# hiroyasuakada/EgoRear

Measured on AMD Instinct MI355X. Metric: 4-view frames/sec (heatmap+MVFEx+3D lift), higher is better.
Workload: dtype f32 (fp16x2 split, 22-bit operands, fp32 accumulate)

## Files before the change

egorear_amd/csrc/egr_pointwise.hip:

```cpp
#include "egr_common.h"
#include <stdlib.h>

namespace {

__global__ __launch_bounds__(256) void maxpool_kernel(const float* x, float* y, int n, int h, int w, int c4, int ho,
                                                      int wo, int k, int stride, int pad) {
    int64_t idx = (int64_t)blockIdx.x * 256 + threadIdx.x;
    int64_t total = (int64_t)n * ho * wo * c4;
    if (idx >= total) return;
    int cq = (int)(idx % c4);
    int64_t p = idx / c4;
    int ox = (int)(p % wo);
    p /= wo;
    int oy = (int)(p % ho);
    int img = (int)(p / ho);
    f32x4 best = {-INFINITY, -INFINITY, -INFINITY, -INFINITY};
    for (int dy = 0; dy < k; ++dy) {
        int iy = oy * stride - pad + dy;
        if (iy < 0 || iy >= h) continue;
        for (int dx = 0; dx < k; ++dx) {
            int ix = ox * stride - pad + dx;
            if (ix < 0 || ix >= w) continue;
            f32x4 v = *reinterpret_cast<const f32x4*>(x + (((int64_t)img * h + iy) * w + ix) * (c4 * 4) + cq * 4);
            best[0] = fmaxf(best[0], v[0]);
// ... 194 lines not shown
    int64_t r = idx / c;
    int jj = (int)(r % j), bb = (int)(r / j);
    if (bpg > 0) embed += (int64_t)(bb / bpg) * j * c;
    y[idx] = (embed[jj * c + ch] + bfb[(int64_t)bb * c + ch]) + hm_embed[idx];
}

__global__ __launch_bounds__(256) void tokens_to_nhwc_kernel(const float* x, float* y, int b, int j, int hw) {
    int64_t idx = (int64_t)blockIdx.x * 256 + threadIdx.x;
    if (idx >= (int64_t)b * j * hw) return;
    int jj = (int)(idx % j);
    int64_t r = idx / j;
    int p = (int)(r % hw), bb = (int)(r / hw);
    y[idx] = x[((int64_t)bb * j + jj) * hw + p];
}


#ifndef HT_ROWS
#define HT_ROWS 8
#endif
constexpr int HT_H = HT_ROWS, HT_W = 32, HT_SRC_H = HT_ROWS / 2 + 2, HT_SRC_W = 18, HT_MAXCO = 16, HT_MAXCIN = 128;
constexpr int HT_RPW = HT_H / 4, HT_NG = 2 * HT_RPW;
typedef float f32x4_mfma __attribute__((ext_vector_type(4)));

template <int CIN>
__global__ __launch_bounds__(256) void up2_relu_head_kernel(const float* lo, int h, int w, int cin_rt, const float* wgt, const float* bias,
                                                            int cout, float* planes, egr_nmap map, int npg, int64_t gy) {
    extern __shared__ __attribute__((aligned(16))) float s_src[];
    const int cin = CIN > 0 ? CIN : cin_rt;
    const int ld = cin + 4;
    const int ho = 2 * h, wo = 2 * w;
    const int tiles_x = wo / HT_W, tiles_y = ho / HT_H;
    int t = blockIdx.x;
    const int img = t / (tiles_x * tiles_y);
    t -= img * tiles_x * tiles_y;
    const int ty = t / tiles_x, tx = t - ty * tiles_x;
    const int oy0 = ty * HT_H, ox0 = tx * HT_W;
    const int grp = img / npg;
    const float sh = (ho > 1) ? (float)(h - 1) / (float)(ho - 1) : 0.f;
    const float sw = (wo > 1) ? (float)(w - 1) / (float)(wo - 1) : 0.f;
    const int sy0 = (int)(sh * (float)oy0), sx0 = (int)(sw * (float)ox0);
    const int c4n = cin >> 2;
    const float* src = lo + (int64_t)img * h * w * cin;
    constexpr int NLD = (HT_SRC_H * HT_SRC_W * (HT_MAXCIN / 4) + 255) / 256;
    f32x4 stg[NLD];
    const int nsrc = HT_SRC_H * HT_SRC_W * c4n;
#pragma unroll
    for (int u = 0; u < NLD; ++u) {
        const int i = threadIdx.x + 256 * u;
        const int ii = i < nsrc ? i : 0;
// ... 52 lines not shown
        }
    };
    const int kblocks = ksteps >> 2;
    fetch(0, 0);
#pragma unroll
    for (int j = 0; j < HT_MAXCIN / 16; ++j) {
        if (j < kblocks) {
            if (j + 1 < kblocks) fetch(j + 1, (j + 1) & 1);
            __builtin_amdgcn_sched_barrier(0);
            f32x4 u[HT_NG];
#pragma unroll
            for (int mg = 0; mg < HT_NG; ++mg) {
                const f32x4* v = sv[j & 1][mg];
                u[mg] = wy0[mg] * (wx0[mg] * v[0] + wx1[mg] * v[1]) + wy1[mg] * (wx0[mg] * v[2] + wx1[mg] * v[3]);
            }
#pragma unroll
            for (int r = 0; r < 4; ++r)
#pragma unroll
                for (int mg = 0; mg < HT_NG; ++mg)
                    acc[mg] = __builtin_amdgcn_mfma_f32_16x16x4f32(fmaxf(u[mg][r], 0.f), bw[4 * j + r], acc[mg], 0, 0, 0);
            __builtin_amdgcn_sched_barrier(0);
        }
    }
    if (pj < cout) {
#pragma unroll
        for (int mg = 0; mg < HT_NG; ++mg) {
            const int oy = oy0 + HT_RPW * wave + (mg >> 1);
            const int oxg = ox0 + (mg & 1) * 16;
            f32x4 v = {acc[mg][0] + bco, acc[mg][1] + bco, acc[mg][2] + bco, acc[mg][3] + bco};
            *reinterpret_cast<f32x4*>(outg + (int64_t)pj * ho * wo + (int64_t)oy * wo + oxg + 4 * kq) = v;
        }
    }
}

constexpr int PT_H = 8, PT_W = 32, PT_SRC_H = PT_H / 2 + 2, PT_SRC_W = 18, PT_NG = 2;
__global__ __launch_bounds__(512) void up2_relu_head_p_kernel(const float* lo, int h, int w, const float* wgt, const float* bias, int cout,
                                                              float* planes, egr_nmap map, int npg, int64_t gy, int ntiles) {
    constexpr int CIN = 128, LD = CIN + 4, C4N = CIN / 4;
    extern __shared__ __attribute__((aligned(16))) float s_src[];
    const int ho = 2 * h, wo = 2 * w;
    const int tiles_x = wo / PT_W, tiles_y = ho / PT_H;
    const float sh = (ho > 1) ? (float)(h - 1) / (float)(ho - 1) : 0.f;
    const float sw = (wo > 1) ? (float)(w - 1) / (float)(wo - 1) : 0.f;
    constexpr int NSRC = PT_SRC_H * PT_SRC_W * C4N;
    constexpr int NLD = (NSRC + 511) / 512;
    f32x4 stg[NLD];
    const int lane = threadIdx.x & 63, wave = threadIdx.x >> 6;
    const int pj = lane & 15, kq = lane >> 4;
    auto decode = [&](int t, int& img, int& oy0, int& ox0) {
        img = t / (tiles_x * tiles_y);
        t -= img * tiles_x * tiles_y;
        const int ty = t / tiles_x, tx = t - ty * tiles_x;
        oy0 = ty * PT_H;
        ox0 = tx * PT_W;
    };
    auto request = [&](int t) {
        int img, oy0, ox0;
        decode(t, img, oy0, ox0);
        const int sy0 = (int)(sh * (float)oy0), sx0 = (int)(sw * (float)ox0);
        const float* src = lo + (int64_t)img * h * w * CIN;
#pragma unroll
        for (int u = 0; u < NLD; ++u) {
            const int i = threadIdx.x + 512 * u;
            const int ii = i < NSRC ? i : 0;
            const int cq = ii % C4N, p = ii / C4N;
            const int py = p / PT_SRC_W, px = p - py * PT_SRC_W;
            const int iy = min(sy0 + py, h - 1), ix = min(sx0 + px, w - 1);
            stg[u] = *reinterpret_cast<const f32x4*>(src + ((int64_t)iy * w + ix) * CIN + cq * 4);
        }
    };
    float bw[CIN / 4];
    float bco = 0.f;
    int cur_grp = -1;
    int tile = blockIdx.x;
    if (tile < ntiles) request(tile);
    for (; tile < ntiles; tile += gridDim.x) {
#pragma unroll
        for (int u = 0; u < NLD; ++u) {
            const int i = threadIdx.x + 512 * u;
            if (i < NSRC) {
                const int cq = i % C4N, p = i / C4N;
                *reinterpret_cast<f32x4*>(&s_src[p * LD + cq * 4]) = stg[u];
            }
        }
        __syncthreads();
        if (tile + (int)gridDim.x < ntiles) request(tile + gridDim.x);
        int img, oy0, ox0;
        decode(tile, img, oy0, ox0);
        const int grp = img / npg;
        if (grp != cur_grp) {
            cur_grp = grp;
            const float* wg = wgt + (int64_t)grp * cout * CIN;
#pragma unroll
            for (int s_ = 0; s_ < CIN / 4; ++s_) bw[s_] = pj < cout ? wg[pj * CIN + 16 * (s_ >> 2) + 4 * kq + (s_ & 3)] : 0.f;
            bco = (bias && pj < cout) ? bias[grp * cout + pj] : 0.f;
        }
        const int sy0 = (int)(sh * (float)oy0), sx0 = (int)(sw * (float)ox0);
        float* outg = planes + grp * gy + egr_map(map, img - grp * npg);
        const float* q00[PT_NG]; const float* q01[PT_NG]; const float* q10[PT_NG]; const float* q11[PT_NG];
        float wy0[PT_NG], wy1[PT_NG], wx0[PT_NG], wx1[PT_NG];
#pragma unroll
        for (int mg = 0; mg < PT_NG; ++mg) {
            const int oy = oy0 + wave;
            const int ox = ox0 + mg * 16 + pj;
            const float fy = sh * (float)oy, fx = sw * (float)ox;
            const int y0 = (int)fy, x0 = (int)fx;
            const int y1 = min(y0 + 1, h - 1), x1 = min(x0 + 1, w - 1);
            wy1[mg] = fminf(fmaxf(fy - (float)y0, 0.f), 1.f); wx1[mg] = fminf(fmaxf(fx - (float)x0, 0.f), 1.f);
            wy0[mg] = 1.f - wy1[mg]; wx0[mg] = 1.f - wx1[mg];
            q00[mg] = s_src + ((y0 - sy0) * PT_SRC_W + (x0 - sx0)) * LD + 4 * kq;
            q01[mg] = s_src + ((y0 - sy0) * PT_SRC_W + (x1 - sx0)) * LD + 4 * kq;
            q10[mg] = s_src + ((y1 - sy0) * PT_SRC_W + (x0 - sx0)) * LD + 4 * kq;
            q11[mg] = s_src + ((y1 - sy0) * PT_SRC_W + (x1 - sx0)) * LD + 4 * kq;
        }
        f32x4_mfma acc[PT_NG];
#pragma unroll
        for (int mg = 0; mg < PT_NG; ++mg) acc[mg] = f32x4_mfma{0.f, 0.f, 0.f, 0.f};
        f32x4 sv[2][PT_NG][4];
        auto fetch = [&](int j, int par) {
#pragma unroll
            for (int mg = 0; mg < PT_NG; ++mg) {
                sv[par][mg][0] = *reinterpret_cast<const f32x4*>(q00[mg] + 16 * j);
                sv[par][mg][1] = *reinterpret_cast<const f32x4*>(q01[mg] + 16 * j);
                sv[par][mg][2] = *reinterpret_cast<const f32x4*>(q10[mg] + 16 * j);
                sv[par][mg][3] = *reinterpret_cast<const f32x4*>(q11[mg] + 16 * j);
            }
        };
        fetch(0, 0);
#pragma unroll
        for (int j = 0; j < CIN / 16; ++j) {
            if (j + 1 < CIN / 16) fetch(j + 1, (j + 1) & 1);
            __builtin_amdgcn_sched_barrier(0);
            f32x4 u[PT_NG];
#pragma unroll
            for (int mg = 0; mg < PT_NG; ++mg) {
                const f32x4* v = sv[j & 1][mg];
                u[mg] = wy0[mg] * (wx0[mg] * v[0] + wx1[mg] * v[1]) + wy1[mg] * (wx0[mg] * v[2] + wx1[mg] * v[3]);
            }
#pragma unroll
            for (int r = 0; r < 4; ++r)
#pragma unroll
                for (int mg = 0; mg < PT_NG; ++mg)
                    acc[mg] = __builtin_amdgcn_mfma_f32_16x16x4f32(fmaxf(u[mg][r], 0.f), bw[4 * j + r], acc[mg], 0, 0, 0);
            __builtin_amdgcn_sched_barrier(0);
        }
        if (pj < cout) {
#pragma unroll
            for (int mg = 0; mg < PT_NG; ++mg) {
                const int oy = oy0 + wave;
                const int oxg = ox0 + mg * 16;
                f32x4 v = {acc[mg][0] + bco, acc[mg][1] + bco, acc[mg][2] + bco, acc[mg][3] + bco};
                *reinterpret_cast<f32x4*>(outg + (int64_t)pj * ho * wo + (int64_t)oy * wo + oxg + 4 * kq) = v;
            }
        }
        __syncthreads();
    }
}

inline unsigned nblocks(int64_t total) { return (unsigned)((total + 255) / 256); }

}

extern "C" int egr_maxpool_nhwc_f32(const float* x, float* y, int32_t n, int32_t h, int32_t w, int32_t c, int32_t k,
                                    int32_t stride, int32_t pad, void* stream) {
    if (!x || !y) return EGR_ENULL;
    if (n <= 0 || c % 4 != 0 || k <= 0 || stride <= 0 || pad < 0 || 2 * pad > k) return EGR_EINVAL;
    int ho = (h + 2 * pad - k) / stride + 1, wo = (w + 2 * pad - k) / stride + 1;
    int64_t total = (int64_t)n * ho * wo * (c / 4);
    if (total <= 0 || total >= (1LL << 31) * 256) return EGR_EINVAL;
    hipLaunchKernelGGL(maxpool_kernel, dim3(nblocks(total)), dim3(256), 0, (hipStream_t)stream, x, y, n, h, w, c / 4, ho,
                       wo, k, stride, pad);
    return egr_launch_status();
}

extern "C" int egr_upsample2x_nhwc_f32(const float* x, int32_t ldx, float* y, int32_t ldy, int32_t n, int32_t h,
                                       int32_t w, int32_t c, int32_t relu, void* stream) {
    if (!x || !y) return EGR_ENULL;
    if (n <= 0 || h <= 0 || w <= 0 || c % 4 != 0 || ldx % 4 != 0 || ldy % 4 != 0 || ldx < c || ldy < c) return EGR_EINVAL;
    const int c4 = c / 4;
    int c4_shift = 0;
    while ((1 << c4_shift) < c4) ++c4_shift;
    if ((1 << c4_shift) != c4) c4_shift = -1;
    if (2 * h > 65535 || (int64_t)h * w * ldx >= (1LL << 31) || (int64_t)2 * w * c4 >= (1LL << 31)) return EGR_EINVAL;
    static const double nt_mb = getenv("EGR_NT_STORE_MB") ? atof(getenv("EGR_NT_STORE_MB")) : 256.0;
    const int nt = ((double)n * 4 * h * w * c * 4.0 >= nt_mb * 1e6) ? 1 : 0;
    for (int n0 = 0; n0 < n; n0 += 65535) {
        const int nn = n - n0 < 65535 ? n - n0 : 65535;
        hipLaunchKernelGGL(upsample2x_kernel, dim3((unsigned)((2 * w * c4 + 255) / 256), (unsigned)h, (unsigned)nn), dim3(256), 0,
                           (hipStream_t)stream, x + (int64_t)n0 * h * w * ldx, ldx, y + (int64_t)n0 * 4 * h * w * ldy, ldy, nn, h, w, c4, c4_shift, relu, nt);
    }
    return egr_launch_status();
}

static int g_head_persist = getenv("EGR_HEAD_PERSIST") ? atoi(getenv("EGR_HEAD_PERSIST")) != 0 : 1;
extern "C" int egr_head_set_persist(int on) {
    const int old = g_head_persist;
    if (on >= 0) g_head_persist = on != 0;
    return old;
}

extern "C" int egr_up2_relu_head_f32(const float* lo, int32_t n, int32_t h, int32_t w, int32_t cin, const float* wgt, const float* bias,
                                     int32_t cout, float* planes, int32_t n_inner, int64_t stride_inner, int64_t stride_outer,
                                     int32_t groups, int64_t gy, void* stream) {
    if (!lo || !wgt || !planes) return EGR_ENULL;
    if (n <= 0 || groups <= 0 || n % groups != 0 || h <= 0 || w <= 0 || cin <= 0 || cin % 16 != 0 || cin > HT_MAXCIN || cout <= 0 ||
        cout > HT_MAXCO || (2 * h) % HT_H != 0 || (2 * w) % HT_W != 0 || n_inner <= 0 || ((uintptr_t)planes & 15) ||
        ((stride_inner | stride_outer | gy) % 4 != 0))
        return EGR_EINVAL;
    egr_nmap map{n_inner, stride_inner, stride_outer};
    const size_t lds = (size_t)(HT_SRC_H * HT_SRC_W * (cin + 4)) * sizeof(float);
    const int64_t blocks = (int64_t)n * ((2 * h) / HT_H) * ((2 * w) / HT_W);
    if (blocks >= (1LL << 31) || lds > 64 * 1024) return EGR_EINVAL;
    if (g_head_persist && cin == 128 && (2 * h) % PT_H == 0 && (2 * w) % PT_W == 0) {
        const int64_t nt = (int64_t)n * ((2 * h) / PT_H) * ((2 * w) / PT_W);
        int dev = 0, cus = 0;
        if (nt >= 1024 && nt < (1LL << 31) && hipGetDevice(&dev) == hipSuccess && dev >= 0 && dev < 64 &&
            hipDeviceGetAttribute(&cus, hipDeviceAttributeMultiprocessorCount, dev) == hipSuccess && cus > 0) {
            const size_t lds_p = (size_t)(PT_SRC_H * PT_SRC_W * (128 + 4)) * sizeof(float);
            static bool allowed[64] = {};
            if (!allowed[dev]) {
                if (hipFuncSetAttribute(reinterpret_cast<const void*>(up2_relu_head_p_kernel), hipFuncAttributeMaxDynamicSharedMemorySize, (int)lds_p) !=
                    hipSuccess)
                    return EGR_EINVAL;
                allowed[dev] = true;
            }
            const unsigned grid = (unsigned)(nt < cus ? nt : cus);
            hipLaunchKernelGGL(up2_relu_head_p_kernel, dim3(grid), dim3(512), lds_p, (hipStream_t)stream, lo, h, w, wgt, bias, cout, planes, map,
                               n / groups, gy, (int)nt);
            return egr_launch_status();
        }
    }
    if (cin == 128)
        hipLaunchKernelGGL(up2_relu_head_kernel<128>, dim3((unsigned)blocks), dim3(256), lds, (hipStream_t)stream, lo, h, w, cin, wgt, bias, cout,
                           planes, map, n / groups, gy);
    else
        hipLaunchKernelGGL(up2_relu_head_kernel<0>, dim3((unsigned)blocks), dim3(256), lds, (hipStream_t)stream, lo, h, w, cin, wgt, bias, cout,
                           planes, map, n / groups, gy);
    return egr_launch_status();
}

__global__ __launch_bounds__(256) void absmax_kernel(const float* __restrict__ x, int64_t n4, int64_t n, unsigned* __restrict__ rec) {
    float m = 0.f;
    const int64_t stride = (int64_t)gridDim.x * 256;
    int64_t i = (int64_t)blockIdx.x * 256 + threadIdx.x;
    for (; i + 7 * stride < n4; i += 8 * stride) {
        f32x4 v[8];
#pragma unroll
        for (int u = 0; u < 8; ++u) v[u] = *reinterpret_cast<const f32x4*>(x + 4 * (i + u * stride));
#pragma unroll
        for (int u = 0; u < 8; ++u) m = fmaxf(m, fmaxf(fmaxf(fabsf(v[u][0]), fabsf(v[u][1])), fmaxf(fabsf(v[u][2]), fabsf(v[u][3]))));
    }
    for (; i < n4; i += stride) {
        const f32x4 v = *reinterpret_cast<const f32x4*>(x + 4 * i);
        m = fmaxf(fmaxf(m, fmaxf(fabsf(v[0]), fabsf(v[1]))), fmaxf(fabsf(v[2]), fabsf(v[3])));
    }
    if (blockIdx.x == 0 && threadIdx.x < (int)(n - 4 * n4)) m = fmaxf(m, fabsf(x[4 * n4 + threadIdx.x]));
    __shared__ float s_m[4];
    m = wave_max(m);
    if ((threadIdx.x & 63) == 0) s_m[threadIdx.x >> 6] = m;
    __syncthreads();
// ... 98 lines not shown
```

egorear_amd/engine.py:

```python
from __future__ import annotations

import math
import os
import threading
from typing import Dict, Optional, Sequence

import numpy as np
import torch
import torch.nn as nn

from . import hip
from .hip import ACT_GELU, ACT_NONE, ACT_RELU, RES_AFTER_ACT, RES_BEFORE_ACT, RES_NONE, RES_UP2_BEFORE_ACT, Img, NMap

_WORKSPACE_FLOATS = 16 << 20



class PConv:
    __slots__ = ("w", "scale", "shift", "cout", "cin", "kh", "kw", "stride", "pad", "groups")


W6_MAX_ELEMS = 1 << 24


# ... 296 lines not shown
                relu2 = k + 1 < len(m0) and isinstance(m0[k + 1], nn.ReLU)
                end = k + (2 if relu2 else 1)
                fin = end >= len(m0)
                ok = (not up) or relu2
                if up and end + 1 == len(m0) and last_kw and "out_nchw" in last_kw:
                    ok = False
                    ph = st.get(nxt, lambda k=k: pack_convs([g[k] for g in mods]))
                    if relu2 and hip.chain_eligible(x, p.w, ph.w, p.cout, ph.cout, p.groups, p.scale, ph.scale):
                        pre_lo = hip.conv1x1_chain(x, p.w, ph.w, p.cout, ph.cout, shift1=p.shift, shift2=ph.shift, act1=act, act2=ACT_NONE,
                                                   groups=p.groups, amax_out=st.new_amax())
                        i = j
                        continue
                if fin and last_kw:
                    ok = False
                p2 = st.get(nxt, lambda k=k: pack_convs([g[k] for g in mods])) if ok else None
                if ok and hip.chain_eligible(x, p.w, p2.w, p.cout, p2.cout, p.groups, p.scale, p2.scale):
                    y = hip.conv1x1_chain(x, p.w, p2.w, p.cout, p2.cout, shift1=p.shift, shift2=p2.shift, act1=act,
                                          act2=ACT_NONE if up else (ACT_RELU if relu2 else ACT_NONE), groups=p.groups,
                                          out=out if (fin and not up) else None, amax_out=st.new_amax())
                    x = hip.upsample2x(y, out=out if fin else None, relu=True) if up else y
                    i = end
                    continue
            kw = dict(last_kw or {}) if last else {}
            if last and out is not None:
                kw["out"] = out
            x = conv(st, x, p, act, **kw)
            i += 2 if act else 1
        elif isinstance(m, nn.Upsample):
            nxt = m0[i + 1] if i + 1 < len(m0) else None
            if (isinstance(nxt, nn.Conv2d) and nxt.kernel_size == (1, 1) and nxt.stride == (1, 1) and i + 2 < len(m0)
                    and isinstance(m0[i + 2], nn.ReLU)):
                p = st.get(nxt, lambda i=i: pack_convs([g[i + 1] for g in mods]))
                lo, pre_lo = (pre_lo, None) if pre_lo is not None else (conv(st, x, p, ACT_NONE), None)
                fin = m0[i + 3] if i + 4 == len(m0) else None
                if (isinstance(fin, nn.Conv2d) and fin.kernel_size == (1, 1) and fin.stride == (1, 1) and fin.out_channels <= 16
                        and fin.in_channels <= 128 and fin.in_channels % 16 == 0 and last_kw is not None and "out_nchw" in last_kw and (2 * lo.h) % 8 == 0
                        and (2 * lo.w) % 32 == 0):
                    wf = st.get((id(fin), "plain"), lambda i=i: (
                        torch.stack([g[i + 3].weight.detach().float().reshape(fin.out_channels, fin.in_channels) for g in mods]).contiguous(),
                        torch.stack([g[i + 3].bias.detach().float() for g in mods]).contiguous() if fin.bias is not None else None))
                    hip.up2_relu_head(lo, wf[0], wf[1], last_kw["out_nchw"], last_kw["ymap"], last_kw.get("gy", 0), groups=len(mods))
                    return None
                last = (i + 3) >= len(m0)
                x = hip.upsample2x(lo, out=out if last else None, relu=True)
                i += 3
            else:
                x = hip.upsample2x(x)
                i += 1
        elif isinstance(m, nn.MaxPool2d):
            k = m.kernel_size if isinstance(m.kernel_size, int) else m.kernel_size[0]
            s = m.stride if isinstance(m.stride, int) else m.stride[0]
            pd = m.padding if isinstance(m.padding, int) else m.padding[0]
            x = hip.maxpool(x, k, s, pd)
            i += 1
        else:
            raise RuntimeError(f"egorear_amd.run_stack: unexpected module {type(m).__name__}")
    return x



def _pack_stems(trunks) -> tuple:
    wps, scs, shs = [], [], []
    for t in trunks:
        conv1, bn = t.layer_s2[0], t.layer_s2[1]
# ... 269 lines not shown
        P.q = {"w_hp2": pk(stk([r.heatmap_proj[2].weight for r in rs])), "b_hp2": stk([r.heatmap_proj[2].bias for r in rs]),
               "w_bfb": pk(stk([r.fc_bfb.weight for r in rs])), "b_bfb": stk([r.fc_bfb.bias for r in rs]),
               "embed": P.embed,
               "w_q": pk(stk([r.fc_query[0].weight for r in rs])), "b_q": stk([r.fc_query[0].bias for r in rs]),
               "w_ol": P.layer.ol_plain["w"], "b_ol": P.layer.ol_plain["b"], "packed": 2 if hip.policy().layer_h2 else True}
    return P


CAPTURE = None


def _run_refiners(st: State, rs, B: int, V: int, hm_init: torch.Tensor, feat_all: torch.Tensor, s32_all: torch.Tensor,
                  anchors, valid, feat_ref: torch.Tensor, hm_ref: torch.Tensor):
    G = len(rs)
    assert G == V
    r0 = rs[0]
    P: PRefiners = st.get(r0, lambda: _pack_refiners(rs))
    J, C = r0.num_heatmap, r0.embed_dims
    hgt, wid = r0.feat_shape
    hw = hgt * wid
    fk = st.fork(G * B)
    with fk:
        ff = run_stack(st, [r.frame_feat_proj_layers for r in rs], Img(feat_all))
    hm_rows = Img(hm_init.view(B * V, J, 1, hw)[0::V])
    t = conv(st, hm_rows, P.hp0, ACT_RELU, gx=J * hw)
    pol = hip.policy()
    fused = pol.fused_layer and P.layer.fused is not None
    ol = None
    if fused and pol.fused_query and P.q is not None and s32_all.shape[-1] == 512:
        x, ol = hip.jqa_query(t.t.view(G * B * J, C), s32_all, P.q, B, J, C, G)
    else:
        hm_embed = linear(st, t.t.view(G * B * J, C), P.hp2)
        bfb = linear(st, hip.avgpool(Img(s32_all)), P.fc_bfb)
        x = linear(st, hip.jqa_sum(hm_embed, P.embed, bfb, G * B, J, C, groups=G), P.fc_query, ACT_RELU)
    head = None
    if fused:
        if pol.fused_query and C == 256 and P.head0_w.shape[1] == 64:
            head = {"w": P.head0_w, "b": P.head0_b, "amax": st.new_amax()}
        _, _, xn, _ = run_layer_fused(st, P.layer, x, feat_all.view(V, B, hw, feat_all.shape[-1]), anchors, valid, B, V, J, hgt, wid, ol=ol,
                                      post={"g": P.post_norm[0], "b": P.post_norm[1]}, want_xn=head is None or CAPTURE is not None, head=head)
    else:
        x = run_layer(st, P.layer, x, feat_all.view(V, B, hw, feat_all.shape[-1]), anchors, valid, B, V, J, hgt, wid)
        xn = hip.layernorm(x, P.post_norm[0], P.post_norm[1], groups=G)
    if head is not None:
        h0 = Img(head["out"])
    else:
        side = int(math.isqrt(C))
# ... 17 lines not shown


@_under_module_policy
def anchors_from_heatmap_api(mod, heatmap):
    a, m, v, _ = _anchors(heatmap.contiguous(), mod.heatmap_threshold)
    return a, m, v.bool()


def _mvfex(mod, img: torch.Tensor, heatmap_for_anchor=None):
    st = _state(mod, img.device)
    st.begin_forward()
    B, V = img.shape[:2]
    img = img.contiguous()
    H4, W4 = img.shape[3] // 4, img.shape[4] // 4
    J = mod.num_heatmap
    dev = img.device
    feat_all = torch.empty((V * B, H4, W4, 128), device=dev, dtype=torch.float32)
    s32_all = torch.empty((V * B, H4 // 8, W4 // 8, 512), device=dev, dtype=torch.float32)
    front, back = mod.heatmap_estimator_stereo_front, mod.heatmap_estimator_stereo_back
    run_backbone(st, [front.encoder, back.encoder], img, 0, 2, Img(feat_all), Img(s32_all))
    hm_init = torch.empty((B, V, J, H4, W4), device=dev, dtype=torch.float32)
    plane = J * H4 * W4
    run_stack(st, [mod.conv_heatmap_layers_stereo_front, mod.conv_heatmap_layers_stereo_back], Img(feat_all),
              last_kw={"out_nchw": hm_init, "ymap": NMap(B, V * plane, plane), "gy": 2 * plane})
    src = heatmap_for_anchor.contiguous() if isinstance(heatmap_for_anchor, torch.Tensor) else hm_init
    anchors, maxvals, valid, index = _anchors(src, mod.heatmap_threshold)
    feat_ref = torch.empty_like(feat_all)
    hm_ref = torch.empty_like(hm_init)
    _run_refiners(st, mod.refiners(), B, V, hm_init, feat_all, s32_all, anchors, valid, feat_ref, hm_ref)
    if CAPTURE is not None:
        CAPTURE.update(feat_init=_vb_view(feat_all, V, B).clone(), feat_refined=_vb_view(feat_ref, V, B).clone())
    aux = {"anchors_2d": anchors, "maxvals": maxvals, "anchors_valid": valid, "argmax_idx": index}
    return hm_init, hm_ref, feat_all, feat_ref, aux


@_under_module_policy
def heatmap_mvfex_forward_api(mod, img, heatmap_for_anchor=None):
    _check_input(img, mod)
    img = as_rgb(img)
    B, V = img.shape[:2]
    hm_init, hm_ref, feat_all, feat_ref, aux = _mvfex(mod, img, heatmap_for_anchor)
    mod.__dict__["_egr_last_aux"] = aux
    return [hm_init, hm_ref], [_vb_view(feat_all, V, B), _vb_view(feat_ref, V, B)]



class PPose:
# ... 151 lines not shown
```

egorear_amd/hip.py:

```python
from __future__ import annotations

import ctypes as C
import os
import threading
from typing import Optional

import torch

_HERE = os.path.dirname(os.path.abspath(__file__))
LIB_PATH = os.environ.get("EGR_LIB") or os.path.join(_HERE, "csrc", "libegorear_hip.so")

ACT_NONE, ACT_RELU, ACT_GELU = 0, 1, 2
RES_NONE, RES_BEFORE_ACT, RES_AFTER_ACT, RES_UP2_BEFORE_ACT = 0, 1, 2, 3



import contextlib
import dataclasses
import sys
import types


@dataclasses.dataclass
class LaunchPolicy:
    w_format: str = "f16x2"
    h2: bool = True
    x6_min_rows: int = 4096
    x6_min_flops: float = 5e8
    x6_train_min_rows: int = 8192
    x6_train_min_flops: float = 4e9
    chain: bool = True
    chain_min_rows: int = 8192
    chain_big: bool = True
    chain_big_min_rows: int = 65536
    wgrad_x6: bool = True
    wgrad_force: bool = False
    layer_h2: bool = True
    fused_layer: bool = True
    fused_query: bool = True

    @classmethod
    def from_env(cls, env=None) -> "LaunchPolicy":
        e = os.environ if env is None else env
        fmt = e.get("EGR_W_FORMAT", "f16x2")
        return cls(w_format=fmt, h2=fmt == "f16x2",
                   x6_min_rows=int(e.get("EGR_X6_MIN_ROWS", "4096")), x6_min_flops=float(e.get("EGR_X6_MIN_FLOPS", "5e8")),
                   x6_train_min_rows=int(e.get("EGR_X6_TRAIN_MIN_ROWS", "8192")), x6_train_min_flops=float(e.get("EGR_X6_TRAIN_MIN_FLOPS", "4e9")),
                   chain=e.get("EGR_CONV_CHAIN", "1") != "0", chain_min_rows=int(e.get("EGR_CONV_CHAIN_MIN_ROWS", "8192")),
                   chain_big=e.get("EGR_CONV_CHAIN_BIG", "1") != "0", chain_big_min_rows=int(e.get("EGR_CONV_CHAIN_BIG_MIN_ROWS", "65536")),
                   wgrad_x6=fmt != "f32", layer_h2=fmt == "f16x2" and e.get("EGR_LAYER_H2", "1") != "0",
                   fused_layer=e.get("EGR_FUSED_LAYER", "1") != "0", fused_query=e.get("EGR_FUSED_QUERY", "1") != "0")

    def replace(self, **kw) -> "LaunchPolicy":
        return dataclasses.replace(self, **kw)

    def pack_key(self) -> tuple:
        return (self.w_format, self.h2, self.layer_h2)

    def exact(self) -> "LaunchPolicy":
        return self.replace(w_format="bf16x3", h2=False, layer_h2=False)


POLICY = LaunchPolicy.from_env()
_POLICY_TLS = threading.local()


def policy() -> LaunchPolicy:
    cur = getattr(_POLICY_TLS, "cur", None)
    return cur if cur is not None else POLICY
# ... 138 lines not shown
    lib.egr_wstream_image_bytes.restype = C.c_int64
    lib.egr_wstream_image_bytes.argtypes = [i32, i32]
    lib.egr_pack_wstream_f32.argtypes = [vp, i32, i32, vp, vp, vp]
    lib.egr_linear_wstream_workspace_bytes.restype = C.c_int64
    lib.egr_linear_wstream_workspace_bytes.argtypes = [i32, i32, i32]
    lib.egr_linear_wstream_f32.argtypes = [vp, i64, i32, i32, vp, vp, vp, i32, i32, vp, vp, i64, vp, vp, i64, vp]
    lib.egr_maxpool_nhwc_f32.argtypes = [vp, vp, i32, i32, i32, i32, i32, i32, i32, vp]
    lib.egr_upsample2x_nhwc_f32.argtypes = [vp, i32, vp, i32, i32, i32, i32, i32, i32, vp]
    lib.egr_avgpool_nhwc_f32.argtypes = [vp, vp, i32, i32, i32, vp]
    lib.egr_argmax_rows_f32.argtypes = [vp, i32, i32, i32, f32, vp, vp, vp, vp, vp]
    lib.egr_layernorm_f32.argtypes = [vp, vp, vp, vp, vp, i32, i32, f32, i32, vp]
    lib.egr_joint_mha_f32.argtypes = [vp, vp, i32, i32, i32, i32, f32, vp]
    lib.egr_msda_gather_f32.argtypes = [vp, i32, vp, i32, vp, vp, vp, i32, i32, i32, i32, i32, i32, vp, vp, vp, vp, i32, vp]
    lib.egr_fisheye_project_f32.argtypes = [vp, vp, vp, i32, i32, vp, vp, vp, vp]
    lib.egr_fisheye_project2_f32.argtypes = [vp, vp, vp, vp, i32, i32, vp, vp, vp, vp]
    lib.egr_linear_smallk_f32.argtypes = [vp, i64, i64, vp, vp, vp, i32, i32, i32, i32, i32, vp]
    lib.egr_jqa_sum_f32.argtypes = [vp, vp, vp, vp, i32, i32, i32, i32, vp]
    lib.egr_tokens_to_nhwc_f32.argtypes = [vp, vp, i32, i32, i32, vp]
    lib.egr_version.restype = C.c_char_p
    lib.egr_w6_elems.restype = C.c_int64
    lib.egr_device_arch.argtypes = [C.c_char_p, i32]
    lib.egr_conv_force_config.argtypes = [i32]
    lib.egr_conv_set_persist.argtypes = [i32, i32]
    lib.egr_up2_relu_head_f32.argtypes = [vp, i32, i32, i32, i32, vp, vp, i32, vp, i32, i64, i64, i32, i64, vp]
    lib.egr_conv2d_masked_f32.argtypes = [C.POINTER(ConvDesc), vp, vp, vp, vp, vp, vp, C.c_size_t, vp]
    lib.egr_conv2d_masked_ex_f32.argtypes = [C.POINTER(ConvDesc), vp, vp, vp, vp, vp, vp, C.c_size_t, C.POINTER(ConvAux), vp]
    lib.egr_conv2d_wgrad_f32.argtypes = [C.POINTER(ConvDesc), vp, vp, vp, vp, vp, C.c_size_t, i32, vp]
    lib.egr_conv2d_wgrad_ex_f32.argtypes = [C.POINTER(ConvDesc), vp, vp, vp, vp, vp, C.c_size_t, i32, vp, vp, vp]
    lib.egr_gt_heatmap_f32.argtypes = [vp, i32, C.c_double, i32, i32, vp, vp, vp]
    lib.egr_pose_metrics_f32.argtypes = [vp, vp, i32, i32, f32, i32, vp, vp, vp]
    lib.egr_heatmap_metrics_f32.argtypes = [C.POINTER(vp), i32, vp, i32, i32, i32, i32, i32, C.POINTER(i32), i32, f32,
                                            vp, vp, vp, vp, vp, vp, vp, vp, vp]
    lib.egr_pack_w6_f32.argtypes = [vp, i32, i32, i32, vp, vp]
    lib.egr_pack_w6_many_f32.argtypes = [vp, i32, i64, vp]
    lib.egr_pack_wh2_many_f32.argtypes = [vp, i32, i64, i64, vp]
    lib.egr_w6_elems.argtypes = [i32, i32]
    lib.egr_msda_fwd_f32.argtypes = [vp, vp, vp, vp, vp, i32, i64, i32, i32, i32, i32, i32, vp, vp]
    lib.egr_msda_bwd_f32.argtypes = [vp, vp, vp, vp, vp, vp, i32, i64, i32, i32, i32, i32, i32, vp, vp, vp, vp]
    lib.egr_joint_layer_f32.argtypes = [C.POINTER(LayerDesc), vp]
    lib.egr_jqa_query_f32.argtypes = [C.POINTER(JqaQueryDesc), vp]
    lib.egr_pose_query_f32.argtypes = [C.POINTER(PoseQueryDesc), vp]
    lib.egr_pack_layer_w_f32.argtypes = [vp, i32, i32, i32, vp, vp]
    lib.egr_pack_layer_wh2_f32.argtypes = [vp, i32, i32, i32, vp, vp]
    lib.egr_preprocess_fused_u8_f32.argtypes = [vp, i32, i32, i32, i32, i32, vp, vp, i32, vp, vp, i32, i32, vp, vp, vp, vp, vp]
    lib.egr_preprocess_band_rows.argtypes = [vp, i32]
    lib.egr_preprocess_u8_f32.argtypes = [vp, i32, i32, i32, i32, i32, vp, vp, i32, vp, vp, i32, vp, vp, vp, vp, vp, vp]
    for name in EXPORTS:
# ... 290 lines not shown
        if gx is None:
            if x.n % groups:
                raise RuntimeError("egorear_amd.conv2d: images not divisible by groups")
            ng = x.n // groups
            gx = ng * x.nstride
            x = Img(x.t[:ng], amax=x.amax)
        ng = x.n
    if transposed_out_hw is not None:
        ho, wo = transposed_out_hw
        if (ho + 2 * pad - kh) // stride + 1 != x.h or (wo + 2 * pad - kw) // stride + 1 != x.w:
            raise RuntimeError("egorear_amd.conv2d: transposed_out_hw inconsistent with dy's size")
    else:
        ho = (x.h + 2 * pad - kh) // stride + 1
        wo = (x.w + 2 * pad - kw) // stride + 1
    npad = (cout + 31) // 32 * 32
    K = kh * kw * x.c
    wshape = (groups, npad, K) if groups > 1 else (npad, K)
    if tuple(w.shape) != wshape:
        raise RuntimeError(f"egorear_amd.conv2d: packed weight shape {tuple(w.shape)} != {wshape}")
    if isinstance(w, W6) and w.f32 is not None:
        rows_all = x.n * groups * ho * wo
        x_bytes = 4 * ((x.n - 1) * x.nstride + (x.h * x.w + 2 * (kh * x.w + kw + 1)) * x.ld) + 64
        min_rows, min_flops = x6_min if x6_min is not None else (pol.x6_min_rows, pol.x6_min_flops)
        if rows_all < min_rows or 2.0 * rows_all * cout * K < min_flops or x_bytes >= (1 << 31):
            w = w.f32
    x6 = isinstance(w, W6)
    if x6 and pol.h2 and w.h2 is not None and x.amax is None and amax_arena is not None and x_full.is_contiguous():
        rec = amax_arena.new()
        if rec is not None:
            absmax_record(x_full, rec)
            x.amax = rec
    h2 = x6 and pol.h2 and w.h2 is not None and x.amax is not None
    if x6 and not h2 and not w.used:
        if w.f32 is not None:
            pack_w6_into(w)
        w.used = True
    if h2 and not w.h2_used:
        if w.f32 is not None:
            pack_wh2_into(w)
        w.h2_used = True
    wptr = (_p(w.h2, torch.float16) if h2 else _p(w.img, torch.bfloat16)) if x6 else _p(_cont(w, "packed weight"))
    d = ConvDesc()
    d.w_format = (4 if h2 else 1) if x6 else 0
    d.n, d.h, d.w, d.cin, d.cout = x.n, x.h, x.w, x.c, cout
    d.kh, d.kw, d.stride, d.pad, d.ho, d.wo = kh, kw, stride, pad, ho, wo
    d.ldx = x.ld
    d.xmap = xmap if xmap is not None else x.nmap()
# ... 353 lines not shown
    ho = (x.h + 2 * pad - k) // stride + 1
    wo = (x.w + 2 * pad - k) // stride + 1
    y = torch.empty((x.n, ho, wo, x.c), device=x.t.device, dtype=torch.float32)
    _launch("egr_maxpool_nhwc_f32", lib.egr_maxpool_nhwc_f32, _p(x.t), _p(y), x.n, x.h, x.w, x.c, k, stride, pad, _stream(),
            nbytes=4.0 * x.n * x.c * (x.h * x.w + ho * wo))
    out = Img(y)
    out.tag(x.amax)
    return out


def upsample2x(x: Img, out: Optional[Img] = None, relu: bool = False) -> Img:
    if x.n > 1 and x.nstride != x.h * x.w * x.ld:
        raise RuntimeError("egorear_amd.upsample2x: images must be densely stacked")
    if out is None:
        out = Img(torch.empty((x.n, 2 * x.h, 2 * x.w, x.c), device=x.t.device, dtype=torch.float32))
    if (out.n, out.h, out.w, out.c) != (x.n, 2 * x.h, 2 * x.w, x.c) or (out.n > 1 and out.nstride != out.h * out.w * out.ld):
        raise RuntimeError("egorear_amd.upsample2x: bad output view")
    _launch("egr_upsample2x_nhwc_f32", lib.egr_upsample2x_nhwc_f32, _p(x.t), x.ld, _p(out.t), out.ld, x.n, x.h, x.w, x.c, 1 if relu else 0, _stream(),
            nbytes=4.0 * 5 * x.n * x.h * x.w * x.c)
    out.tag(x.amax)
    return out


def up2_relu_head(lo: Img, wgt: torch.Tensor, bias: Optional[torch.Tensor], planes: torch.Tensor, ymap: NMap, gy: int, groups: int = 1):
    if not lo.t.is_contiguous() or lo.n % groups:
        raise RuntimeError("egorear_amd.up2_relu_head: dense NHWC input with groups | n expected")
    cout, cin = wgt.shape[-2], wgt.shape[-1]
    npg = lo.n // groups
    if cin != lo.c or wgt.numel() != groups * cout * cin or (bias is not None and bias.numel() != groups * cout):
        raise RuntimeError("egorear_amd.up2_relu_head: weight / bias shape")
    ho, wo = 2 * lo.h, 2 * lo.w
    last = (groups - 1) * gy + (npg - 1) // ymap.n_inner * ymap.stride_outer + min(npg - 1, ymap.n_inner - 1) * ymap.stride_inner + cout * ho * wo
    if not planes.is_contiguous() or last > planes.numel():
        raise RuntimeError("egorear_amd.up2_relu_head: output map runs outside the tensor")
    _launch("egr_up2_relu_head_f32", lib.egr_up2_relu_head_f32, _p(lo.t), lo.n, lo.h, lo.w, cin, _p(_cont(wgt, "weight")), _p(bias), cout,
            _p(planes), ymap.n_inner, ymap.stride_inner, ymap.stride_outer, groups, gy, _stream(),
            flops=2.0 * lo.n * ho * wo * cout * cin, nbytes=4.0 * lo.n * (lo.h * lo.w * cin + cout * ho * wo))


def avgpool(x: Img) -> torch.Tensor:
    if not x.t.is_contiguous():
        raise RuntimeError("egorear_amd.avgpool: contiguous input expected")
    y = torch.empty((x.n, x.c), device=x.t.device, dtype=torch.float32)
    _launch("egr_avgpool_nhwc_f32", lib.egr_avgpool_nhwc_f32, _p(x.t), _p(y), x.n, x.h * x.w, x.c, _stream(),
            nbytes=4.0 * x.n * x.c * (x.h * x.w + 1))
    return y


def argmax_rows(hm: torch.Tensor, thr: float):
    _cont(hm, "heatmap")
    H, W = hm.shape[-2:]
    rows = hm.numel() // (H * W)
    dev = hm.device
    anchors = torch.empty((rows, 2), device=dev, dtype=torch.float32)
    maxvals = torch.empty((rows,), device=dev, dtype=torch.float32)
    valid = torch.empty((rows,), device=dev, dtype=torch.uint8)
    index = torch.empty((rows,), device=dev, dtype=torch.int32)
    _launch("egr_argmax_rows_f32", lib.egr_argmax_rows_f32, _p(hm), rows, H, W, float(thr), _p(anchors), _p(maxvals), _p(valid, torch.uint8),
                                   _p(index, torch.int32), _stream(), nbytes=4.0 * hm.numel() + 17.0 * rows)
    return anchors, maxvals, valid, index
# ... 286 lines not shown
```

include/egorear_hip.h:

```cpp
#ifndef EGOREAR_HIP_H
#define EGOREAR_HIP_H

#include <stddef.h>
#include <stdint.h>

#ifdef __cplusplus
extern "C" {
#endif

#define EGR_EINVAL (-1)
#define EGR_ENULL (-2)
#define EGR_EWORKSPACE (-3)

enum { EGR_ACT_NONE = 0, EGR_ACT_RELU = 1, EGR_ACT_GELU = 2 };
enum { EGR_RES_NONE = 0, EGR_RES_BEFORE_ACT = 1, EGR_RES_AFTER_ACT = 2,
       EGR_RES_UP2_BEFORE_ACT = 3  };

typedef struct {
    int32_t n_inner;
    int64_t stride_inner;
    int64_t stride_outer;
} egr_nmap;

typedef struct {
// ... 94 lines not shown
    int32_t reduce_pass;
    int32_t bn_slabs;
} egr_conv_plan_t;
int egr_conv_plan(const egr_conv_desc* d, const float* x, const void* w, const float* scale, const float* shift,
                  const float* res, const float* rowscale, const uint8_t* rowmask, const float* mask, const float* y,
                  const float* workspace, size_t workspace_floats, const egr_conv_aux* aux, egr_conv_plan_t* out);

int egr_conv2d_wgrad_f32(const egr_conv_desc* d, const float* x, const float* dy, float* dw, float* db,
                         float* workspace, size_t workspace_floats, int32_t accumulate, void* stream);
int egr_conv2d_wgrad_ex_f32(const egr_conv_desc* d, const float* x, const float* dy, float* dw, float* db, float* workspace,
                            size_t workspace_floats, int32_t accumulate, const uint32_t* amax_x, const uint32_t* amax_dy, void* stream);
int egr_wgrad_last_h2(void);
int egr_wgrad_last_kernel(void);

int egr_conv_force_config(int cfg);
int egr_conv_last_kernel(void);
int egr_conv_set_splitk_fused(int on);
int egr_conv_set_tap(int on);
int egr_conv_set_tapx(int32_t on, int32_t min_tiles, int32_t blocks);
int egr_conv_set_persist(int slots, int max_ktiles);

int egr_up2_relu_head_f32(const float* lo, int32_t n, int32_t h, int32_t w, int32_t cin, const float* wgt, const float* bias,
                          int32_t cout, float* planes, int32_t n_inner, int64_t stride_inner, int64_t stride_outer,
                          int32_t groups, int64_t gy, void* stream);
int egr_head_set_persist(int on);

int egr_conv_debug_stamps(unsigned long long* buf);

int egr_stem_conv7x7_f32(const float* x, egr_nmap xmap, int32_t n, int32_t h, int32_t w,
                         const float* wpack, const float* scale, const float* shift, float* y,
                         int32_t groups ,
                         int64_t gx, void* stream);

int egr_stem_conv7x7_pool_f32(const float* x, egr_nmap xmap, int32_t n, int32_t h, int32_t w,
                              const float* wpack, const float* scale, const float* shift, float* y,
                              int32_t groups, int64_t gx, void* stream);

int64_t egr_stem_w6_bytes(void);
int egr_pack_stem_w6_f32(const float* w, int32_t groups, void* w6, void* stream);
int egr_stem_conv7x7_x6_f32(const float* x, egr_nmap xmap, int32_t n, int32_t h, int32_t w,
                            const void* w6, const float* scale, const float* shift, float* y,
                            int32_t pool, int32_t groups, int64_t gx, void* stream);
int egr_stem_conv7x7_x6_ex_f32(const float* x, egr_nmap xmap, int32_t n, int32_t h, int32_t w,
                            const void* w6, const float* scale, const float* shift, float* y,
                            int32_t pool, int32_t groups, int64_t gx, uint32_t* amax_out, void* stream);
int64_t egr_wstream_image_bytes(int32_t n, int32_t k);
int egr_pack_wstream_f32(const float* w, int32_t n, int32_t k, void* img, float* descale, void* stream);
// ... 140 lines not shown
```

Before: 6925.

## Fuse amax into head kernel, deepen head tile pipelining, enable h2 path for deep 1x1

```diff
diff --git a/egorear_amd/csrc/egr_pointwise.hip b/egorear_amd/csrc/egr_pointwise.hip
--- a/egorear_amd/csrc/egr_pointwise.hip
+++ b/egorear_amd/csrc/egr_pointwise.hip
@@ -240,9 +240,15 @@
 constexpr int HT_RPW = HT_H / 4, HT_NG = 2 * HT_RPW;
 typedef float f32x4_mfma __attribute__((ext_vector_type(4)));
 
+__device__ __forceinline__ void head_amax_flush(unsigned* amax, float amx, int slot) {
+    amx = wave_max(amx);
+    if ((threadIdx.x & 63) == 0 && amx > 0.f)
+        __hip_atomic_fetch_max(amax + (slot & 63), __float_as_uint(amx), __ATOMIC_RELAXED, __HIP_MEMORY_SCOPE_AGENT);
+}
+
 template <int CIN>
 __global__ __launch_bounds__(256) void up2_relu_head_kernel(const float* lo, int h, int w, int cin_rt, const float* wgt, const float* bias,
-                                                            int cout, float* planes, egr_nmap map, int npg, int64_t gy) {
+                                                            int cout, float* planes, egr_nmap map, int npg, int64_t gy, unsigned* amax) {
     extern __shared__ __attribute__((aligned(16))) float s_src[];
     const int cin = CIN > 0 ? CIN : cin_rt;
     const int ld = cin + 4;
@@ -341,6 +347,7 @@
             __builtin_amdgcn_sched_barrier(0);
         }
     }
+    float amx = 0.f;
     if (pj < cout) {
 #pragma unroll
         for (int mg = 0; mg < HT_NG; ++mg) {
@@ -348,14 +355,19 @@
             const int oxg = ox0 + (mg & 1) * 16;
             f32x4 v = {acc[mg][0] + bco, acc[mg][1] + bco, acc[mg][2] + bco, acc[mg][3] + bco};
             *reinterpret_cast<f32x4*>(outg + (int64_t)pj * ho * wo + (int64_t)oy * wo + oxg + 4 * kq) = v;
-        }
-    }
-}
-
-constexpr int PT_H = 8, PT_W = 32, PT_SRC_H = PT_H / 2 + 2, PT_SRC_W = 18, PT_NG = 2;
+            amx = fmaxf(amx, fmaxf(fmaxf(fabsf(v[0]), fabsf(v[1])), fmaxf(fabsf(v[2]), fabsf(v[3]))));
+        }
+    }
+    if (amax) head_amax_flush(amax, amx, (int)blockIdx.x * 4 + wave);
+}
+
+#ifndef HEAD_VALU_PER_MFMA
+#define HEAD_VALU_PER_MFMA 4
+#endif
+constexpr int PT_H = 16, PT_W = 32, PT_SRC_H = PT_H / 2 + 2, PT_SRC_W = 18, PT_NG = 4;
 __global__ __launch_bounds__(512) void up2_relu_head_p_kernel(const float* lo, int h, int w, const float* wgt, const float* bias, int cout,
-                                                              float* planes, egr_nmap map, int npg, int64_t gy, int ntiles) {
-    constexpr int CIN = 128, LD = CIN + 4, C4N = CIN / 4;
+                                                              float* planes, egr_nmap map, int npg, int64_t gy, int ntiles, unsigned* amax) {
+    constexpr int CIN = 128, LD = CIN + 4, C4N = CIN / 4, KB = CIN / 16;
     extern __shared__ __attribute__((aligned(16))) float s_src[];
     const int ho = 2 * h, wo = 2 * w;
     const int tiles_x = wo / PT_W, tiles_y = ho / PT_H;
@@ -390,6 +402,7 @@
     };
     float bw[CIN / 4];
     float bco = 0.f;
+    float amx = 0.f;
     int cur_grp = -1;
     int tile = blockIdx.x;
     if (tile < ntiles) request(tile);
@@ -416,64 +429,78 @@
         }
         const int sy0 = (int)(sh * (float)oy0), sx0 = (int)(sw * (float)ox0);
         float* outg = planes + grp * gy + egr_map(map, img - grp * npg);
-        const float* q00[PT_NG]; const float* q01[PT_NG]; const float* q10[PT_NG]; const float* q11[PT_NG];
-        float wy0[PT_NG], wy1[PT_NG], wx0[PT_NG], wx1[PT_NG];
-#pragma unroll
-        for (int mg = 0; mg < PT_NG; ++mg) {
-            const int oy = oy0 + wave;
-            const int ox = ox0 + mg * 16 + pj;
+        float wy0[2], wy1[2], wx0[2], wx1[2];
+        int yo0[2], yo1[2], xo0[2], xo1[2];
+#pragma unroll
+        for (int i = 0; i < 2; ++i) {
+            const int oy = oy0 + 2 * wave + i;
+            const int ox = ox0 + i * 16 + pj;
             const float fy = sh * (float)oy, fx = sw * (float)ox;
             const int y0 = (int)fy, x0 = (int)fx;
             const int y1 = min(y0 + 1, h - 1), x1 = min(x0 + 1, w - 1);
-            wy1[mg] = fminf(fmaxf(fy - (float)y0, 0.f), 1.f); wx1[mg] = fminf(fmaxf(fx - (float)x0, 0.f), 1.f);
-            wy0[mg] = 1.f - wy1[mg]; wx0[mg] = 1.f - wx1[mg];
-            q00[mg] = s_src + ((y0 - sy0) * PT_SRC_W + (x0 - sx0)) * LD + 4 * kq;
-            q01[mg] = s_src + ((y0 - sy0) * PT_SRC_W + (x1 - sx0)) * LD + 4 * kq;
-            q10[mg] = s_src + ((y1 - sy0) * PT_SRC_W + (x0 - sx0)) * LD + 4 * kq;
-            q11[mg] = s_src + ((y1 - sy0) * PT_SRC_W + (x1 - sx0)) * LD + 4 * kq;
+            wy1[i] = fminf(fmaxf(fy - (float)y0, 0.f), 1.f); wx1[i] = fminf(fmaxf(fx - (float)x0, 0.f), 1.f);
+            wy0[i] = 1.f - wy1[i]; wx0[i] = 1.f - wx1[i];
+            yo0[i] = (y0 - sy0) * PT_SRC_W * LD; yo1[i] = (y1 - sy0) * PT_SRC_W * LD;
+            xo0[i] = (x0 - sx0) * LD + 4 * kq;   xo1[i] = (x1 - sx0) * LD + 4 * kq;
         }
         f32x4_mfma acc[PT_NG];
 #pragma unroll
         for (int mg = 0; mg < PT_NG; ++mg) acc[mg] = f32x4_mfma{0.f, 0.f, 0.f, 0.f};
-        f32x4 sv[2][PT_NG][4];
-        auto fetch = [&](int j, int par) {
+        f32x4 sv[PT_NG][4];
+        f32x4 u[2][PT_NG];
+        auto fetch = [&](int j, int mg) {
+            const int r = mg >> 1, c = mg & 1;
+            sv[mg][0] = *reinterpret_cast<const f32x4*>(s_src + yo0[r] + xo0[c] + 16 * j);
+            sv[mg][1] = *reinterpret_cast<const f32x4*>(s_src + yo0[r] + xo1[c] + 16 * j);
+            sv[mg][2] = *reinterpret_cast<const f32x4*>(s_src + yo1[r] + xo0[c] + 16 * j);
+            sv[mg][3] = *reinterpret_cast<const f32x4*>(s_src + yo1[r] + xo1[c] + 16 * j);
+        };
+        auto interp = [&](int par, int mg) {
+            const int r = mg >> 1, c = mg & 1;
+            const f32x4* v = sv[mg];
+            const f32x4 t = wy0[r] * (wx0[c] * v[0] + wx1[c] * v[1]) + wy1[r] * (wx0[c] * v[2] + wx1[c] * v[3]);
+            u[par][mg] = f32x4{fmaxf(t[0], 0.f), fmaxf(t[1], 0.f), fmaxf(t[2], 0.f), fmaxf(t[3], 0.f)};
+        };
+#pragma unroll
+        for (int mg = 0; mg < PT_NG; ++mg) fetch(0, mg);
+#pragma unroll
+        for (int mg = 0; mg < PT_NG; ++mg) {
+            interp(0, mg);
+            fetch(1, mg);
+        }
+#pragma unroll
+        for (int j = 0; j < KB; ++j) {
+#pragma unroll
+            for (int r = 0; r < 4; ++r) {
+                __builtin_amdgcn_sched_barrier(0);
+#pragma unroll
+                for (int mg = 0; mg < PT_NG; ++mg)
+                    acc[mg] = __builtin_amdgcn_mfma_f32_16x16x4f32(u[j & 1][mg][r], bw[4 * j + r], acc[mg], 0, 0, 0);
+                if (j + 1 < KB) {
+                    interp((j + 1) & 1, r);
+                    if (j + 2 < KB) fetch(j + 2, r);
+#pragma unroll
+                    for (int i = 0; i < 4; ++i) {
+                        __builtin_amdgcn_sched_group_barrier(0x8, 1, 0);
+                        __builtin_amdgcn_sched_group_barrier(0x2, HEAD_VALU_PER_MFMA, 0);
+                    }
+                }
+            }
+        }
+        __builtin_amdgcn_sched_barrier(0);
+        if (pj < cout) {
 #pragma unroll
             for (int mg = 0; mg < PT_NG; ++mg) {
-                sv[par][mg][0] = *reinterpret_cast<const f32x4*>(q00[mg] + 16 * j);
-                sv[par][mg][1] = *reinterpret_cast<const f32x4*>(q01[mg] + 16 * j);
-                sv[par][mg][2] = *reinterpret_cast<const f32x4*>(q10[mg] + 16 * j);
-                sv[par][mg][3] = *reinterpret_cast<const f32x4*>(q11[mg] + 16 * j);
-            }
-        };
-        fetch(0, 0);
-#pragma unroll
-        for (int j = 0; j < CIN / 16; ++j) {
-            if (j + 1 < CIN / 16) fetch(j + 1, (j + 1) & 1);
-            __builtin_amdgcn_sched_barrier(0);
-            f32x4 u[PT_NG];
-#pragma unroll
-            for (int mg = 0; mg < PT_NG; ++mg) {
-                const f32x4* v = sv[j & 1][mg];
-                u[mg] = wy0[mg] * (wx0[mg] * v[0] + wx1[mg] * v[1]) + wy1[mg] * (wx0[mg] * v[2] + wx1[mg] * v[3]);
-            }
-#pragma unroll
-            for (int r = 0; r < 4; ++r)
-#pragma unroll
-                for (int mg = 0; mg < PT_NG; ++mg)
-                    acc[mg] = __builtin_amdgcn_mfma_f32_16x16x4f32(fmaxf(u[mg][r], 0.f), bw[4 * j + r], acc[mg], 0, 0, 0);
-            __builtin_amdgcn_sched_barrier(0);
-        }
-        if (pj < cout) {
-#pragma unroll
-            for (int mg = 0; mg < PT_NG; ++mg) {
-                const int oy = oy0 + wave;
-                const int oxg = ox0 + mg * 16;
+                const int oy = oy0 + 2 * wave + (mg >> 1);
+                const int oxg = ox0 + (mg & 1) * 16;
                 f32x4 v = {acc[mg][0] + bco, acc[mg][1] + bco, acc[mg][2] + bco, acc[mg][3] + bco};
                 *reinterpret_cast<f32x4*>(outg + (int64_t)pj * ho * wo + (int64_t)oy * wo + oxg + 4 * kq) = v;
+                amx = fmaxf(amx, fmaxf(fmaxf(fabsf(v[0]), fabsf(v[1])), fmaxf(fabsf(v[2]), fabsf(v[3]))));
             }
         }
         __syncthreads();
     }
+    if (amax) head_amax_flush(amax, amx, (int)blockIdx.x * 8 + wave);
 }
 
 inline unsigned nblocks(int64_t total) { return (unsigned)((total + 255) / 256); }
@@ -520,8 +547,9 @@
 
 extern "C" int egr_up2_relu_head_f32(const float* lo, int32_t n, int32_t h, int32_t w, int32_t cin, const float* wgt, const float* bias,
                                      int32_t cout, float* planes, int32_t n_inner, int64_t stride_inner, int64_t stride_outer,
-                                     int32_t groups, int64_t gy, void* stream) {
+                                     int32_t groups, int64_t gy, uint32_t* amax, void* stream) {
     if (!lo || !wgt || !planes) return EGR_ENULL;
+    if ((uintptr_t)amax & 3) return EGR_EINVAL;
     if (n <= 0 || groups <= 0 || n % groups != 0 || h <= 0 || w <= 0 || cin <= 0 || cin % 16 != 0 || cin > HT_MAXCIN || cout <= 0 ||
         cout > HT_MAXCO || (2 * h) % HT_H != 0 || (2 * w) % HT_W != 0 || n_inner <= 0 || ((uintptr_t)planes & 15) ||
         ((stride_inner | stride_outer | gy) % 4 != 0))
@@ -545,16 +573,16 @@
             }
             const unsigned grid = (unsigned)(nt < cus ? nt : cus);
             hipLaunchKernelGGL(up2_relu_head_p_kernel, dim3(grid), dim3(512), lds_p, (hipStream_t)stream, lo, h, w, wgt, bias, cout, planes, map,
-                               n / groups, gy, (int)nt);
+                               n / groups, gy, (int)nt, amax);
             return egr_launch_status();
         }
     }
     if (cin == 128)
         hipLaunchKernelGGL(up2_relu_head_kernel<128>, dim3((unsigned)blocks), dim3(256), lds, (hipStream_t)stream, lo, h, w, cin, wgt, bias, cout,
-                           planes, map, n / groups, gy);
+                           planes, map, n / groups, gy, amax);
     else
         hipLaunchKernelGGL(up2_relu_head_kernel<0>, dim3((unsigned)blocks), dim3(256), lds, (hipStream_t)stream, lo, h, w, cin, wgt, bias, cout,
-                           planes, map, n / groups, gy);
+                           planes, map, n / groups, gy, amax);
     return egr_launch_status();
 }
 
diff --git a/egorear_amd/engine.py b/egorear_amd/engine.py
--- a/egorear_amd/engine.py
+++ b/egorear_amd/engine.py
@@ -342,6 +342,7 @@
                     i = end
                     continue
             kw = dict(last_kw or {}) if last else {}
+            kw.pop("head_amax", None)
             if last and out is not None:
                 kw["out"] = out
             x = conv(st, x, p, act, **kw)
@@ -359,7 +360,8 @@
                     wf = st.get((id(fin), "plain"), lambda i=i: (
                         torch.stack([g[i + 3].weight.detach().float().reshape(fin.out_channels, fin.in_channels) for g in mods]).contiguous(),
                         torch.stack([g[i + 3].bias.detach().float() for g in mods]).contiguous() if fin.bias is not None else None))
-                    hip.up2_relu_head(lo, wf[0], wf[1], last_kw["out_nchw"], last_kw["ymap"], last_kw.get("gy", 0), groups=len(mods))
+                    hip.up2_relu_head(lo, wf[0], wf[1], last_kw["out_nchw"], last_kw["ymap"], last_kw.get("gy", 0), groups=len(mods),
+                                      amax_out=last_kw.get("head_amax"))
                     return None
                 last = (i + 3) >= len(m0)
                 x = hip.upsample2x(lo, out=out if last else None, relu=True)
@@ -675,7 +677,7 @@
     fk = st.fork(G * B)
     with fk:
         ff = run_stack(st, [r.frame_feat_proj_layers for r in rs], Img(feat_all))
-    hm_rows = Img(hm_init.view(B * V, J, 1, hw)[0::V])
+    hm_rows = Img(hm_init.view(B * V, J, 1, hw)[0::V], amax=getattr(hm_init, "_egr_amax", None))
     t = conv(st, hm_rows, P.hp0, ACT_RELU, gx=J * hw)
     pol = hip.policy()
     fused = pol.fused_layer and P.layer.fused is not None
@@ -739,7 +741,7 @@
     hm_init = torch.empty((B, V, J, H4, W4), device=dev, dtype=torch.float32)
     plane = J * H4 * W4
     run_stack(st, [mod.conv_heatmap_layers_stereo_front, mod.conv_heatmap_layers_stereo_back], Img(feat_all),
-              last_kw={"out_nchw": hm_init, "ymap": NMap(B, V * plane, plane), "gy": 2 * plane})
+              last_kw={"out_nchw": hm_init, "ymap": NMap(B, V * plane, plane), "gy": 2 * plane, "head_amax": st.new_amax()})
     src = heatmap_for_anchor.contiguous() if isinstance(heatmap_for_anchor, torch.Tensor) else hm_init
     anchors, maxvals, valid, index = _anchors(src, mod.heatmap_threshold)
     feat_ref = torch.empty_like(feat_all)
diff --git a/egorear_amd/hip.py b/egorear_amd/hip.py
--- a/egorear_amd/hip.py
+++ b/egorear_amd/hip.py
@@ -27,6 +27,7 @@
     h2: bool = True
     x6_min_rows: int = 4096
     x6_min_flops: float = 5e8
+    h2_deep_min_rows: int = 3072
     x6_train_min_rows: int = 8192
     x6_train_min_flops: float = 4e9
     chain: bool = True
@@ -45,6 +46,7 @@
         fmt = e.get("EGR_W_FORMAT", "f16x2")
         return cls(w_format=fmt, h2=fmt == "f16x2",
                    x6_min_rows=int(e.get("EGR_X6_MIN_ROWS", "4096")), x6_min_flops=float(e.get("EGR_X6_MIN_FLOPS", "5e8")),
+                   h2_deep_min_rows=int(e.get("EGR_H2_DEEP_MIN_ROWS", "3072")),
                    x6_train_min_rows=int(e.get("EGR_X6_TRAIN_MIN_ROWS", "8192")), x6_train_min_flops=float(e.get("EGR_X6_TRAIN_MIN_FLOPS", "4e9")),
                    chain=e.get("EGR_CONV_CHAIN", "1") != "0", chain_min_rows=int(e.get("EGR_CONV_CHAIN_MIN_ROWS", "8192")),
                    chain_big=e.get("EGR_CONV_CHAIN_BIG", "1") != "0", chain_big_min_rows=int(e.get("EGR_CONV_CHAIN_BIG_MIN_ROWS", "65536")),
@@ -229,7 +231,7 @@
     lib.egr_device_arch.argtypes = [C.c_char_p, i32]
     lib.egr_conv_force_config.argtypes = [i32]
     lib.egr_conv_set_persist.argtypes = [i32, i32]
-    lib.egr_up2_relu_head_f32.argtypes = [vp, i32, i32, i32, i32, vp, vp, i32, vp, i32, i64, i64, i32, i64, vp]
+    lib.egr_up2_relu_head_f32.argtypes = [vp, i32, i32, i32, i32, vp, vp, i32, vp, i32, i64, i64, i32, i64, vp, vp]
     lib.egr_conv2d_masked_f32.argtypes = [C.POINTER(ConvDesc), vp, vp, vp, vp, vp, vp, C.c_size_t, vp]
     lib.egr_conv2d_masked_ex_f32.argtypes = [C.POINTER(ConvDesc), vp, vp, vp, vp, vp, vp, C.c_size_t, C.POINTER(ConvAux), vp]
     lib.egr_conv2d_wgrad_f32.argtypes = [C.POINTER(ConvDesc), vp, vp, vp, vp, vp, C.c_size_t, i32, vp]
@@ -566,7 +568,9 @@
         rows_all = x.n * groups * ho * wo
         x_bytes = 4 * ((x.n - 1) * x.nstride + (x.h * x.w + 2 * (kh * x.w + kw + 1)) * x.ld) + 64
         min_rows, min_flops = x6_min if x6_min is not None else (pol.x6_min_rows, pol.x6_min_flops)
-        if rows_all < min_rows or 2.0 * rows_all * cout * K < min_flops or x_bytes >= (1 << 31):
+        deep = (x6_min is None and pol.h2 and w.h2 is not None and x.amax is not None and kh == 1 and kw == 1 and K >= 2048
+                and rows_all >= pol.h2_deep_min_rows)
+        if (rows_all < min_rows and not deep) or 2.0 * rows_all * cout * K < min_flops or x_bytes >= (1 << 31):
             w = w.f32
     x6 = isinstance(w, W6)
     if x6 and pol.h2 and w.h2 is not None and x.amax is None and amax_arena is not None and x_full.is_contiguous():
@@ -966,7 +970,10 @@
     return out
 
 
-def up2_relu_head(lo: Img, wgt: torch.Tensor, bias: Optional[torch.Tensor], planes: torch.Tensor, ymap: NMap, gy: int, groups: int = 1):
+def up2_relu_head(lo: Img, wgt: torch.Tensor, bias: Optional[torch.Tensor], planes: torch.Tensor, ymap: NMap, gy: int, groups: int = 1,
+                  amax_out: Optional[torch.Tensor] = None):
+    if amax_out is not None and (amax_out.numel() != 64 or amax_out.dtype != torch.int32 or not amax_out.is_contiguous()):
+        raise RuntimeError("egorear_amd.up2_relu_head: amax_out must be 64 contiguous int32 slots")
     if not lo.t.is_contiguous() or lo.n % groups:
         raise RuntimeError("egorear_amd.up2_relu_head: dense NHWC input with groups | n expected")
     cout, cin = wgt.shape[-2], wgt.shape[-1]
@@ -978,8 +985,9 @@
     if not planes.is_contiguous() or last > planes.numel():
         raise RuntimeError("egorear_amd.up2_relu_head: output map runs outside the tensor")
     _launch("egr_up2_relu_head_f32", lib.egr_up2_relu_head_f32, _p(lo.t), lo.n, lo.h, lo.w, cin, _p(_cont(wgt, "weight")), _p(bias), cout,
-            _p(planes), ymap.n_inner, ymap.stride_inner, ymap.stride_outer, groups, gy, _stream(),
+            _p(planes), ymap.n_inner, ymap.stride_inner, ymap.stride_outer, groups, gy, _p(amax_out, torch.int32), _stream(),
             flops=2.0 * lo.n * ho * wo * cout * cin, nbytes=4.0 * lo.n * (lo.h * lo.w * cin + cout * ho * wo))
+    planes._egr_amax = amax_out
 
 
 def avgpool(x: Img) -> torch.Tensor:
diff --git a/include/egorear_hip.h b/include/egorear_hip.h
--- a/include/egorear_hip.h
+++ b/include/egorear_hip.h
@@ -140,7 +140,7 @@
 
 int egr_up2_relu_head_f32(const float* lo, int32_t n, int32_t h, int32_t w, int32_t cin, const float* wgt, const float* bias,
                           int32_t cout, float* planes, int32_t n_inner, int64_t stride_inner, int64_t stride_outer,
-                          int32_t groups, int64_t gy, void* stream);
+                          int32_t groups, int64_t gy, uint32_t* amax, void* stream);
 int egr_head_set_persist(int on);
 
 int egr_conv_debug_stamps(unsigned long long* buf);
```

Result: no change. 6944, median of 2 (+0.3%).
